# jonH34400/3DBodyAnimation

Measured on AMD Instinct MI355X. Metric: SMPL residual+Jacobian evals/sec (6890v, 10 beta, 24 joints), higher is better.
Workload: dtype f64 residual/Jacobian; f32 mesh (f32 + split-bf16 MFMA blend); 1 GPU; C3: 256 independent frames per GPU, BODY_25 (14 FK joints + 11 vertex landmarks), opt-shape (per-frame beta, 86 cols), GMM prior on, 6890-vertex mesh on; frames_per_gpu=256, keypoints_per_frame=25, n_cols=86

## Files before the change

3dbodyanimation_amd/csrc/frame_part_inl.h:

```cpp
#pragma once
#include <hip/hip_ext.h>

#include "bodyfit_device.h"
#include "priors_inl.h"

namespace bodyfit {
namespace {

__device__ __forceinline__ void store_through(double* p, double v) {
  __hip_atomic_store(p, v, __ATOMIC_RELAXED, __HIP_MEMORY_SCOPE_SYSTEM);
}
#ifndef BODYFIT_J_THROUGH
#define BODYFIT_J_THROUGH 1
#endif
template <bool kFused>
__device__ __forceinline__ void store_J(double* p, double v, int scope = 0) {
  if constexpr (kFused && !BODYFIT_J_THROUGH) *p = v;
  else if (scope == 1) store_f64_through(p, v);
  else if (scope == 2) *p = v;
  else store_through(p, v);
}


__device__ inline void mul33(const double* A, const double* B, double* C) {
#pragma unroll
  for (int r = 0; r < 3; ++r)
#pragma unroll
    for (int c = 0; c < 3; ++c) C[r * 3 + c] = A[r * 3] * B[c] + A[r * 3 + 1] * B[3 + c] + A[r * 3 + 2] * B[6 + c];
}
__device__ inline void mul33_bt(const double* A, const double* B, double* C) {
#pragma unroll
  for (int r = 0; r < 3; ++r)
#pragma unroll
    for (int c = 0; c < 3; ++c)
      C[r * 3 + c] = A[r * 3] * B[c * 3] + A[r * 3 + 1] * B[c * 3 + 1] + A[r * 3 + 2] * B[c * 3 + 2];
}
// ... 119 lines not shown
struct FusedFrame {
  unsigned* flag;
  unsigned epoch;
  int j_scope;
};

template <bool kFused>
__device__ __forceinline__ void frame_sync() {
  if constexpr (kFused) asm volatile("s_waitcnt lgkmcnt(0)\n\ts_barrier" ::: "memory");
  else __syncthreads();
}

template <bool kFused>
__device__ __forceinline__ void store_operand16(void* p, uint4 v) {
  if constexpr (kFused) {
    typedef __attribute__((ext_vector_type(4))) unsigned int u32x4_;
    const u32x4_ x = {v.x, v.y, v.z, v.w};
    asm volatile("global_store_dwordx4 %0, %1, off sc1\n\ts_nop 1" ::"v"(p), "v"(x) : "memory");
  } else {
    *reinterpret_cast<uint4*>(p) = v;
  }
}

template <bool kFused>
__device__ __forceinline__ void frame_part(const DevModel& M, const DevProblem& Pb, const double* __restrict__ params,
                                           const double* __restrict__ beta, double* __restrict__ r_out,
                                           double* __restrict__ J_out, double* __restrict__ joints_out, const MeshCoef& mc,
                                           int want_jac, double* sm, int f, const FusedFrame& fu, const FrameHead& hd) {
  const int tid = threadIdx.x;
  const int lane = tid & 63, wave = tid >> 6;
  const int nJ = kFused ? (hd.dims & 63) : M.nJ, nS = kFused ? ((hd.dims >> 6) & 15) : M.nS, nL = kFused ? ((hd.dims >> 10) & 63) : M.nL;
  const int ncols = kFused ? ((hd.dims >> 16) & 255) : Pb.ncols;
  const int npose = 7 + 3 * (nJ - 1);
  const bool use_shape = kFused ? (((hd.dims >> 24) & 1) != 0) : (Pb.use_shape != 0);
  const int beta_stride = kFused ? ((hd.dims >> 25) & 15) : Pb.beta_stride;
  const unsigned char* const mtab = kFused ? hd.mtab : M.tabA;
  const unsigned char* const ptab = kFused ? hd.ptab : Pb.ptab;
  const int* const t_parent = reinterpret_cast<const int*>(mtab + kTabParent);
  const unsigned* const t_anc = reinterpret_cast<const unsigned*>(mtab + kTabAnc);
  const unsigned long long* const t_chain = reinterpret_cast<const unsigned long long*>(mtab + kTabChain);
  const int* const t_lm_woff = reinterpret_cast<const int*>(mtab + kTabLmWoff);
  const int* const t_lm_wj = reinterpret_cast<const int*>(mtab + kTabLmWj);
  const double* const t_lm_ww = reinterpret_cast<const double*>(mtab + kTabLmWw);
  const double* const t_lm_vt = reinterpret_cast<const double*>(mtab + kTabLmVt);
  const double* const t_lm_sd = reinterpret_cast<const double*>(mtab + kTabLmSd);
  const double* const t_dS = reinterpret_cast<const double*>(mtab + kTabDS);
  const double* const t_Sc = reinterpret_cast<const double*>(mtab + kTabSc);
  const double* const t_offset = reinterpret_cast<const double*>(mtab + kTabOffset);
  const double* const t_Jc0 = reinterpret_cast<const double*>(mtab + kTabJc0);
  const int t_F = kFused ? hd.F : Pb.F, t_K = kFused ? hd.K : Pb.K;
  const int* const t_kp_offset = reinterpret_cast<const int*>(ptab);
  const int* const t_kp_id = reinterpret_cast<const int*>(ptab + ptab_id_off(t_F));
  const double* const t_kp_uv = reinterpret_cast<const double*>(ptab + ptab_uv_off(t_F, t_K));
  const double* const t_R0 = kFused ? hd.R0 : Pb.R0;
  const int P = M.P;
  double* sx = sm + OFF_X;
  double* sR = sm + OFF_R;
  double* sdR = sm + OFF_DR;
// ... 580 lines not shown
    }
  }
  double* sJb = sdR;
  double fold_acc = 0.0;
  typedef __attribute__((ext_vector_type(4))) double fold_d4;
  fold_d4 fold_gram = {0.0, 0.0, 0.0, 0.0};
  for (int kc0 = k_begin; kc0 < k_end; kc0 += KC) {
    const int nk = min(KC, k_end - kc0);
    frame_sync<kFused>();
    if (kc0 != k_begin) {
      if (tid < nk) stage_kp(tid, kc0);
      frame_sync<kFused>();
    }
    STAMP(7);
    if (want_jac) {
      const int njc = npose - 7;
      const int ngrp = kThreads / njc;
      if (tid < ngrp * njc) {
        const int g = tid / njc, kc = tid - g * njc, k = 1 + kc / 3;
        double Wm[9];
#pragma unroll
        for (int e9 = 0; e9 < 9; ++e9) Wm[e9] = sW[kc * 9 + e9];
        const double pk0 = sP[k * 3], pk1 = sP[k * 3 + 1], pk2 = sP[k * 3 + 2];
        for (int kk = g; kk < nk; kk += ngrp) {
          const int kg = kc0 + kk;
          const int id = sKpId[kk];
          const unsigned am = sKpAnc[kk];
          const double* kp = sKp + kk * 18;
          const double* G = kp + 12;
          double d0 = 0.0, d1 = 0.0, d2 = 0.0;
          if (id < nJ) {
            if ((am >> k) & 1u) {
              const double x0 = kp[0] - pk0, x1 = kp[1] - pk1, x2 = kp[2] - pk2;
              d0 = Wm[0] * x0 + Wm[1] * x1 + Wm[2] * x2;
              d1 = Wm[3] * x0 + Wm[4] * x1 + Wm[5] * x2;
              d2 = Wm[6] * x0 + Wm[7] * x1 + Wm[8] * x2;
            }
          } else {
            const double* o = sLm + (id - nJ) * LM_STRIDE + LM_PD + kc * 3;
            d0 = o[0]; d1 = o[1]; d2 = o[2];
          }
          store_J<kFused>(J_out + (size_t)(2 * kg) * ncols + 7 + kc, G[0] * d0 + G[1] * d1 + G[2] * d2, fu.j_scope);
          store_J<kFused>(J_out + (size_t)(2 * kg + 1) * ncols + 7 + kc, G[3] * d0 + G[4] * d1 + G[5] * d2, fu.j_scope);
        }
      }
      const int nsc = 7 + (ncols - npose);
      for (int e = tid; e < nk * nsc; e += kThreads) {
        const int kk = e / nsc, c = e - kk * nsc;
        const int kg = kc0 + kk;
        const int id = sKpId[kk];
        const double* kp = sKp + kk * 18;
        const double* G = kp + 12;
        double j0, j1;
        int col;
        if (c == 0) {
          col = 0;
          j0 = kp[6] * kp[3] + kp[7] * kp[4] + kp[8] * kp[5];
          j1 = kp[9] * kp[3] + kp[10] * kp[4] + kp[11] * kp[5];
        } else if (c < 4) {
          col = c;
          double t[3];
          mv3(dRr0 + (c - 1) * 9, kp[0], kp[1], kp[2], t);
          j0 = s * (kp[6] * t[0] + kp[7] * t[1] + kp[8] * t[2]);
          j1 = s * (kp[9] * t[0] + kp[10] * t[1] + kp[11] * t[2]);
        } else if (c < 7) {
          col = c;
          j0 = kp[6 + (c - 4)];
          j1 = kp[9 + (c - 4)];
        } else {
          const int k = c - 7;
          col = npose + k;
          double d0 = 0.0, d1 = 0.0, d2 = 0.0;
          if (use_shape) {
            if (id < nJ) {
              if (id == 0 || sParent[id] < 0) {
                d0 = sDS[(id * 3 + 0) * nS + k]; d1 = sDS[(id * 3 + 1) * nS + k]; d2 = sDS[(id * 3 + 2) * nS + k];
              } else {
                d0 = sB[(id * 3 + 0) * nS + k]; d1 = sB[(id * 3 + 1) * nS + k]; d2 = sB[(id * 3 + 2) * nS + k];
              }
            } else {
              const double* o = sLm + (id - nJ) * LM_STRIDE + LM_BETA + k * 3;
              d0 = o[0]; d1 = o[1]; d2 = o[2];
            }
          }
          j0 = G[0] * d0 + G[1] * d1 + G[2] * d2;
          j1 = G[3] * d0 + G[4] * d1 + G[5] * d2;
        }
        store_J<kFused>(J_out + (size_t)(2 * kg) * ncols + col, j0, fu.j_scope);
        store_J<kFused>(J_out + (size_t)(2 * kg + 1) * ncols + col, j1, fu.j_scope);
        if (fold && c >= 7) { sJb[(2 * kk) * kMaxShape + c - 7] = j0; sJb[(2 * kk + 1) * kMaxShape + c - 7] = j1; }
      }
    }
    if (fold) {
      frame_sync<kFused>();
      if (wave == 0) {
        const int col = lane & 15, kq = lane >> 4;
        for (int s0 = 0; s0 < (2 * nk + 3) / 4; s0 += 4) {
          double vv[4];
#pragma unroll
          for (int u = 0; u < 4; ++u) {
            const int row = 4 * (s0 + u) + kq;
            const bool on = row < 2 * nk;
            const double sw = on ? sFeat[row >> 1] : 0.0;
            const double x = (on && col < nS) ? sJb[row * kMaxShape + col] : ((on && col == 10) ? sKpUv[row] : 0.0);
            vv[u] = sw * x;
          }
#pragma unroll
          for (int u = 0; u < 4; ++u) fold_gram = __builtin_amdgcn_mfma_f64_16x16x4f64(vv[u], vv[u], fold_gram, 0, 0, 0);
        }
      } else if (tid == 64) {
        for (int kk = 0; kk < nk; ++kk) fold_acc += sFeat[KC + kk];
      }
    }
  }
// ... 24 lines not shown
```

3dbodyanimation_amd/csrc/k_sweep.hip:

```cpp
#include <hip/hip_ext.h>

#include "bodyfit_device.h"
#include "frame_part_inl.h"
#include "mesh_part_inl.h"
#include "mesh_role_inl.h"
#include "priors_inl.h"

namespace bodyfit {
namespace {

[[maybe_unused]] constexpr int kPollWave = 7;

__global__ __launch_bounds__(kThreads, 4) void k_frame_resjac(DevModel M, DevProblem Pb, const double* __restrict__ params,
                                                      const double* __restrict__ beta, double* __restrict__ r_out,
                                                      double* __restrict__ J_out, double* __restrict__ joints_out,
                                                      MeshCoef mc, int want_jac, PriorArgs pa) {
  extern __shared__ __attribute__((aligned(16))) double sm[];
  if ((int)blockIdx.x < pa.n_tiles) {
#ifdef BODYFIT_STAMPS
    unsigned long long tp0 = 0;
    if (Pb.dbg && threadIdx.x == 0) asm volatile("s_memrealtime %0\n\ts_waitcnt lgkmcnt(0)" : "=s"(tp0)::"memory");
#endif
    if (Pb.frame_flags) {
      const int f = (int)blockIdx.x * kPriorTileF + (int)(threadIdx.x & 15);
// ... 96 lines not shown
    out66[tid] = v;
  }
}

struct RoleArgs {
  DevModel M;
  DevProblem Pb;
  const double* params;
  const double* beta;
  double* r_out;
  double* J_out;
  double* joints_out;
  MeshCoef mc;
  int want_jac;
  PriorArgs pa;
  float* cloud_f;
  FusedSync sy;
  FoldTail fold;
};
typedef const __attribute__((address_space(4))) RoleArgs* RoleArgP;

static_assert(alignof(RoleArgs) == 8, "kernel-argument segment: 4 ints, 5 pointers, then RoleArgs at offset 56");
[[maybe_unused]] constexpr int kRoleArgsOffset = 4 * 4 + 5 * 8;
__global__ __launch_bounds__(kThreads, 4) void k_sweep_roles(int F_arg, int nVT_arg, int K_arg, int dims_arg,
                                                             const unsigned char* __restrict__ mtab_arg,
                                                             const unsigned char* __restrict__ ptab_arg,
                                                             const double* __restrict__ R0_arg, const double* __restrict__ params_arg,
                                                             const double* __restrict__ beta_arg, RoleArgs by_value) {
  (void)by_value;
#if defined(__HIP_DEVICE_COMPILE__)
  extern __shared__ __attribute__((aligned(16))) unsigned char lds[];
  const RoleArgP A =
      (RoleArgP)((const __attribute__((address_space(4))) unsigned char*)__builtin_amdgcn_kernarg_segment_ptr() + kRoleArgsOffset);
  const int F = F_arg, nVT = nVT_arg;
  int role = 2, idx = 0, grp = 0;
  {
    const int nG = (F + kRoleGroup - 1) / kRoleGroup;
    int pos = (int)blockIdx.x;
    const int n0 = min(kRoleGroup, F);
    if (pos < n0) { role = 0; idx = pos; }
    else {
      pos -= n0;
      bool found = false;
      for (int g = 1; g < nG && !found; ++g) {
        const int ng = min(kRoleGroup, F - kRoleGroup * g);
        if (pos < ng) { role = 0; idx = kRoleGroup * g + pos; found = true; }
        else {
          pos -= ng;
          if (pos < nVT) { role = 1; idx = pos; grp = g - 1; found = true; }
          else pos -= nVT;
        }
      }
      if (!found) {
        if (pos < nVT) { role = 1; idx = pos; grp = nG - 1; }
        else { role = 2; idx = pos - nVT; }
      }
    }
  }
  if (role == 0) {
    const DevModel M = A->M;
    const DevProblem Pb = A->Pb;
    const MeshCoef mc = A->mc;
    FusedFrame fu;
    fu.flag = A->sy.flag;
    fu.epoch = A->sy.epoch;
    fu.j_scope = A->sy.j_scope;
    __builtin_amdgcn_s_setprio(2);
    FrameHead hd;
    hd.mtab = mtab_arg; hd.ptab = ptab_arg; hd.R0 = R0_arg; hd.F = F_arg; hd.K = K_arg; hd.dims = dims_arg;
    frame_part<true>(M, Pb, params_arg, beta_arg, A->r_out, A->J_out, A->joints_out, mc, A->want_jac,
                     reinterpret_cast<double*>(lds), idx, fu, hd);
    if (A->fold.ticket)
      fold_tail(A->fold.ticket, A->fold.want, A->fold.n_partials, A->fold.partials, A->fold.beta, A->fold.shape_rows,
                A->fold.beta_shape, A->fold.out66, lds);
    return;
  }
  const unsigned epoch = A->sy.epoch;
  const unsigned long long kRoleTimeoutTicks = A->sy.timeout_ticks;
  unsigned* const flag_base = A->sy.flag;
  unsigned* const error_word = A->sy.error;
  if (role == 2) grp = (idx * kPriorTileF) / kRoleGroup;
  const unsigned max_polls = (unsigned)min(kRoleTimeoutTicks / 110ull, 0x7fffffffull);
  auto wait_flags = [&]() {
    const int tid = threadIdx.x, lane = tid & 63;
    if ((tid >> 6) == kPollWave) {
      const int fbeg = grp * kRoleGroup, nf = min(kRoleGroup, F - fbeg);
      const int nu = (nf + kFTile - 1) / kFTile;
      const unsigned want = epoch * (unsigned)min(kFTile, nf - min(lane, 7) * kFTile);
      const unsigned* ctr = flag_base + (size_t)(grp * (kRoleGroup / kFTile) + min(lane, 7)) * kUnitCounterStride;
      const unsigned long long t_enter = __builtin_amdgcn_s_memrealtime();
      for (unsigned polls = 0;; ++polls) {
        const unsigned got = __hip_atomic_load(ctr, __ATOMIC_RELAXED, __HIP_MEMORY_SCOPE_AGENT);
        if (__all(lane >= nu || got == want)) break;
        if (polls >= max_polls) break;
// ... 19 lines not shown
  const DevModel M = A->M;
  const DevProblem Pb = A->Pb;
  const MeshCoef mc = A->mc;
  const unsigned long long t_role = __builtin_amdgcn_s_memrealtime();
  const int my_unit = __builtin_amdgcn_readfirstlane(threadIdx.x >> 6);
  const unsigned want = epoch * (unsigned)max(0, min(kFTile, F - (grp * kRoleGroup + my_unit * kFTile)));
  const unsigned* ctr = flag_base + (size_t)(grp * (kRoleGroup / kFTile) + my_unit) * kUnitCounterStride;
  auto wait_unit = [&](const unsigned* c) -> bool {
    for (unsigned polls = 0;; ++polls) {
      const unsigned got = __hip_atomic_load(c, __ATOMIC_RELAXED, __HIP_MEMORY_SCOPE_AGENT);
      if (got == want) return true;
      if (polls >= max_polls) return false;
      if (__builtin_amdgcn_s_memrealtime() - t_role < 300) {
        for (int i = 0; i < 6 && __builtin_amdgcn_s_memrealtime() - t_role < 300; ++i) __builtin_amdgcn_s_sleep(20);
      } else {
        __builtin_amdgcn_s_sleep(9);
      }
    }
  };
  auto fail = [&]() {
    if (threadIdx.x == 0) __hip_atomic_store(error_word, 1u, __ATOMIC_RELAXED, __HIP_MEMORY_SCOPE_AGENT);
  };
  mesh_role(M, Pb, mc, A->cloud_f, idx, grp, lds, (int)blockIdx.x < A->sy.resident_blocks, ctr, want, wait_unit, fail,
            A->sy.mesh_prio_early, A->sy.trickle_start, A->sy.trickle_sleep);
#endif
}

}

void launch_frame_resjac(const DevModel& M, const DevProblem& P, const double* d_params, const double* d_beta,
                         double* d_r, double* d_J, double* d_joints, const MeshCoef& mc, int want_jac,
                         const PriorArgs& priors, hipStream_t s, hipEvent_t ev_start, hipEvent_t ev_stop) {
  if (P.F <= 0) return;
  const size_t lds = frame_lds_bytes(M.nL);
  static DeviceMax lds_granted;
  lds_granted.raise(current_device(), lds, 48 * 1024, [&](size_t want) {
    (void)hipFuncSetAttribute(reinterpret_cast<const void*>(k_frame_resjac), hipFuncAttributeMaxDynamicSharedMemorySize,
                              (int)want);
  });
  BODYFIT_LAUNCH_EXT(k_frame_resjac, dim3(P.F + priors.n_tiles), dim3(kThreads), lds, s, ev_start, ev_stop, 0, M, P,
                        d_params, d_beta, d_r, d_J, d_joints, mc, want_jac, priors);
}

void launch_mesh(const DevModel& M, const DevProblem& P, const MeshCoef& mc, float* d_cloud, const PriorArgs& pa,
                 const double* d_params, hipStream_t s, hipEvent_t ev_start, hipEvent_t ev_stop) {
  if (P.F <= 0) return;
  if ((size_t)P.nFTiles * kFTile * M.nVTiles * kVTile * 12 >= ((size_t)1 << 32)) return;
  static DeviceOnce attr;
  attr.run(current_device(), [&] {
    (void)hipFuncSetAttribute(reinterpret_cast<const void*>(k_mesh_blend_lbs),
                              hipFuncAttributeMaxDynamicSharedMemorySize, kLdsBytes);
  });
  BODYFIT_LAUNCH_EXT(k_mesh_blend_lbs, dim3(M.nVTiles + pa.n_tiles), dim3(64 * kWaves), kLdsBytes, s, ev_start, ev_stop,
                        0, M, P, mc, d_cloud, pa, d_params);
}

bool role_sweep_fits(const DevModel& M, const DevProblem& P) {
  return P.F > 0 && P.F <= kRoleMaxFrames && M.nVTiles > 0 && frame_lds_bytes(M.nL) <= (size_t)kRoleLdsBytes &&
         (size_t)P.nFTiles * kFTile * M.nVTiles * kVTile * 12 < ((size_t)1 << 32);
}

void launch_sweep_roles(const DevModel& M, const DevProblem& P, const double* d_params, const double* d_beta, double* d_r,
                        double* d_J, double* d_joints, const MeshCoef& mc, int want_jac, const PriorArgs& pa, float* d_cloud,
                        const FusedSync& sy, const FoldTail& fold, hipStream_t s, hipEvent_t ev_start, hipEvent_t ev_stop) {
  static DeviceOnce attr;
  attr.run(current_device(), [&] {
    (void)hipFuncSetAttribute(reinterpret_cast<const void*>(k_sweep_roles), hipFuncAttributeMaxDynamicSharedMemorySize,
                              kRoleLdsBytes);
  });
  const int nG = (P.F + kRoleGroup - 1) / kRoleGroup;
  const int grid = P.F + nG * M.nVTiles + pa.n_tiles;
  RoleArgs A;
  A.M = M; A.Pb = P; A.Pb.feat_perm = 1; A.params = d_params; A.beta = d_beta; A.r_out = d_r; A.J_out = d_J;
  A.joints_out = d_joints; A.mc = mc; A.want_jac = want_jac; A.pa = pa; A.cloud_f = d_cloud; A.sy = sy; A.fold = fold;
  const int dims = frame_head_dims(M.nJ, M.nS, M.nL, P.ncols, P.use_shape, P.beta_stride, mc.featA != nullptr);
  BODYFIT_LAUNCH_EXT(k_sweep_roles, dim3(grid), dim3(kThreads), kRoleLdsBytes, s, ev_start, ev_stop, 0, P.F, M.nVTiles, P.K, dims,
                     M.tabA, P.ptab, P.R0, d_params, d_beta, A);
}

}
```

3dbodyanimation_amd/csrc/mesh_role_inl.h:

```cpp
#pragma once
#include <hip/hip_ext.h>

#include "bodyfit_device.h"
#include "mesh_part_inl.h"

namespace bodyfit {
namespace {

constexpr int kRoleGroup = 256;
constexpr int kSlabBytes = 3 * 2 * 1024;
constexpr int kResident = 13;
constexpr int kRegionASlabs = 4;
constexpr int kRegionABytes = kRegionASlabs * kSlabBytes;
constexpr int kRegionTSlabs = kResident - kRegionASlabs;
constexpr int kTRowBytes = 2 * kRowBytes;
constexpr int kTRing = 4;
constexpr int kTWaveBytes = 3 * kTRowBytes;
constexpr int kTSlot3Bytes = kRegionABytes / kWaves;
constexpr int kRoleCtrlOff = kRegionABytes + kWaves * kTWaveBytes;
constexpr int kRoleLdsBytes = kRoleCtrlOff + 16;
constexpr int kLoadSc1 = 16;
static_assert(kRegionTSlabs * kSlabBytes == kWaves * kTWaveBytes, "the transform rings take over region T exactly");
static_assert(kTSlot3Bytes >= kTRowBytes, "ring slot 3");
static_assert(kRoleLdsBytes <= 80 * 1024, "two workgroups per CU");
__host__ __device__ constexpr int role_slab_off(int s) {
  return s < kRegionTSlabs ? kRegionABytes + s * kSlabBytes : (s - kRegionTSlabs) * kSlabBytes;
}

typedef __attribute__((address_space(3))) unsigned char lds_u8;
typedef __attribute__((ext_vector_type(4))) float f32x4;
typedef const __attribute__((address_space(3))) u32x4 lds_u32x4;
typedef const __attribute__((address_space(3))) f32x4 lds_f32x4;

#ifdef BODYFIT_STAMPS
#define RSTAMP(i)                                                                                              \
  do {                                                                                                         \
    if (Pb.dbg && C.lane == 0) {                                                                               \
      unsigned long long t_;                                                                                   \
      asm volatile("s_memrealtime %0\n\ts_waitcnt lgkmcnt(0)" : "=s"(t_)::"memory");                          \
      Pb.dbg[kStampBase + ((size_t)(group * M.nVTiles + vtile) * 8 + C.wave) * 16 + (i)] = t_;                 \
    }                                                                                                          \
  } while (0)
#define RCYC(i)                                                                                                \
  do {                                                                                                         \
// ... 31 lines not shown
};

__device__ __forceinline__ void role_dma_slab(const RoleCtx& C, int s) {
  __builtin_amdgcn_raw_ptr_buffer_load_lds(C.dirs_rsrc, (__attribute__((address_space(3))) void*)(C.ring + role_slab_off(s) + C.piece * 1024),
                                       16, C.slab_voff, C.dirs_soff + (unsigned)s * kSlabBytes, 0, 0);
}
__device__ __forceinline__ void role_dma_row(const RoleCtx& C, int r) {
  const unsigned so = C.skin_soff + (unsigned)r * kTRowBytes;
  lds_u8* l = (r % kTRing) == 3 ? C.trow3 : C.trow + (r % kTRing) * kTRowBytes;
  __builtin_amdgcn_raw_ptr_buffer_load_lds(C.skin_rsrc, (__attribute__((address_space(3))) void*)l, 16, C.lane * 16, so, 0, kLoadSc1);
  __builtin_amdgcn_raw_ptr_buffer_load_lds(C.skin_rsrc, (__attribute__((address_space(3))) void*)(l + 1024), 16, C.lane * 16, so + 1024, 0, kLoadSc1);
  __builtin_amdgcn_raw_ptr_buffer_load_lds(C.skin_rsrc, (__attribute__((address_space(3))) void*)(l + 2048), 4, C.lane * 4, so + 2048, 0, kLoadSc1);
}

template <int S>
__device__ __forceinline__ void role_blend_step(const RoleCtx& C, const __amdgpu_buffer_rsrc_t& feat_rsrc, unsigned feat_off,
                                                f32x16 (&acc)[3], u32x4 (&a)[3][2], u32x4 (&bq)[3][2]) {
  const bf16x8 a_hi = __builtin_bit_cast(bf16x8, a[S % 3][0]);
  const bf16x8 a_lo = __builtin_bit_cast(bf16x8, a[S % 3][1]);
#pragma unroll
  for (int c = 0; c < 3; ++c) {
    const bf16x8 bhi = __builtin_bit_cast(bf16x8, bq[c][0]);
    const bf16x8 blo = __builtin_bit_cast(bf16x8, bq[c][1]);
    if constexpr (S == 0) {
      f32x16 z;
#pragma unroll
      for (int r = 0; r < 16; ++r) z[r] = 0.0f;
      acc[c] = __builtin_amdgcn_mfma_f32_32x32x16_bf16(a_hi, bhi, z, 0, 0, 0);
    } else {
      acc[c] = __builtin_amdgcn_mfma_f32_32x32x16_bf16(a_hi, bhi, acc[c], 0, 0, 0);
    }
    acc[c] = __builtin_amdgcn_mfma_f32_32x32x16_bf16(a_hi, blo, acc[c], 0, 0, 0);
    acc[c] = __builtin_amdgcn_mfma_f32_32x32x16_bf16(a_lo, bhi, acc[c], 0, 0, 0);
    if constexpr (S + 1 < kResident && S + 1 != kRegionTSlabs) {
      const unsigned sl = C.ring_addr + (unsigned)(role_slab_off(S + 1) + (c * 2) * 1024);
      bq[c][0] = *(lds_u32x4*)(size_t)(sl);
      bq[c][1] = *(lds_u32x4*)(size_t)(sl + 1024u);
    } else if constexpr (S + 1 >= kResident && S + 1 < kBlendKSteps) {
      const unsigned so = C.dirs_soff + (unsigned)((S + 1) * kSlabBytes + (c * 2) * 1024);
      bq[c][0] = __builtin_amdgcn_raw_buffer_load_b128(C.dirs_rsrc, (unsigned)(C.lane * 16), so, 0);
      bq[c][1] = __builtin_amdgcn_raw_buffer_load_b128(C.dirs_rsrc, (unsigned)(C.lane * 16), so + 1024, 0);
    }
  }
  if constexpr (S + 3 < kBlendKSteps) {
    const unsigned soff = feat_off + (unsigned)((S + 3) * 2 * 1024);
    a[S % 3][0] = __builtin_amdgcn_raw_buffer_load_b128(feat_rsrc, feat_frag_off(C.lane, 0), soff, kLoadSc1);
    a[S % 3][1] = __builtin_amdgcn_raw_buffer_load_b128(feat_rsrc, feat_frag_off(C.lane, 1), soff, kLoadSc1);
  }
#pragma unroll
  for (int c = 0; c < 3; ++c) {
    __builtin_amdgcn_sched_group_barrier(0x008, 3, 0);
    if constexpr (S + 1 < kResident && S + 1 != kRegionTSlabs) __builtin_amdgcn_sched_group_barrier(0x100, 2, 0);
    else if constexpr (S + 1 >= kResident && S + 1 < kBlendKSteps) __builtin_amdgcn_sched_group_barrier(0x020, 2, 0);
  }
  if constexpr (S + 3 < kBlendKSteps) __builtin_amdgcn_sched_group_barrier(0x020, 2, 0);
  __builtin_amdgcn_sched_barrier(0);
}

template <int R>
__device__ __forceinline__ void role_skin_row(const RoleCtx& C, const RoleLane& L, const f32x16 (&acc)[3],
                                              __amdgpu_buffer_rsrc_t cloud, unsigned row_off) {
  if constexpr (R >= 3) ROLE_WAIT_VM(role_skin_ops(R - 3) + role_skin_ops(R - 2) + role_skin_ops(R - 1));
  const unsigned slot = (R % kTRing) == 3 ? L.slot3 : (unsigned)(R % kTRing) * kTRowBytes;
  f32x4 t[12];
  const unsigned tj[4] = {L.tj0, L.tj1, L.tj2, L.tj3};
  const float wgt[4] = {L.w0, L.w1, L.w2, L.w3};
#pragma unroll
  for (int i = 0; i < 4; ++i) {
    lds_f32x4* T = (lds_f32x4*)(tj[i] + slot);
    t[3 * i + 0] = T[0]; t[3 * i + 1] = T[1]; t[3 * i + 2] = T[2];
  }
  f32x2 b[6];
  const f32x2 w0 = {wgt[0], wgt[0]};
#pragma unroll
  for (int k = 0; k < 3; ++k) {
    b[2 * k] = w0 * f32x2{t[k].x, t[k].y};
    b[2 * k + 1] = w0 * f32x2{t[k].z, t[k].w};
  }
// ... 5 lines not shown
      b[2 * k] += wi * f32x2{t[3 * i + k].x, t[3 * i + k].y};
      b[2 * k + 1] += wi * f32x2{t[3 * i + k].z, t[3 * i + k].w};
    }
  }
  const f32x2 pxy = {acc[0][R], acc[1][R]};
  const f32x2 pz1 = {acc[2][R], 1.0f};
  typedef __attribute__((ext_vector_type(3))) unsigned int u32x3;
  u32x3 pk;
#pragma unroll
  for (int k = 0; k < 3; ++k) {
    const f32x2 m = b[2 * k] * pxy + b[2 * k + 1] * pz1;
    pk[k] = __float_as_uint(m.x + m.y);
  }
  __builtin_amdgcn_raw_buffer_store_b96(pk, cloud, L.out_off, row_off, kStoreAux);
  if constexpr (R + kTRing < 16) role_dma_row(C, R + kTRing);
  asm volatile("" ::: "memory");
}


template <typename WaitUnit, typename Fail>
__device__ __forceinline__ void mesh_role(const DevModel& M, const DevProblem& Pb, const MeshCoef& mc, float* __restrict__ cloud_f,
                                          int vtile, int group, unsigned char* lds_generic, bool beside_its_frames,
                                          const unsigned* unit_ctr, unsigned unit_want, WaitUnit wait_unit, Fail fail,
                                          int prio_early, int trickle_start, int trickle_sleep) {
  RoleCtx C;
  C.wave = __builtin_amdgcn_readfirstlane(threadIdx.x >> 6);
  C.lane = threadIdx.x & 63;
  lds_u8* lds = (lds_u8*)lds_generic;
  C.ring = lds;
  C.ring_addr = (unsigned)(size_t)lds + (unsigned)C.lane * 16u;
  C.trow = lds + kRegionABytes + C.wave * kTWaveBytes;
  C.trow3 = lds + C.wave * kTSlot3Bytes;
  C.dirs_rsrc = __builtin_amdgcn_make_buffer_rsrc(const_cast<uint16_t*>(M.dirsB), 0, M.nVTiles * kBBytes, 0x00020000);
  C.dirs_soff = (unsigned)vtile * kBBytes;
  const int nFT = Pb.nFTiles;
  const int ftile = group * (kRoleGroup / kFTile) + C.wave;
  const bool active = ftile < nFT;
  const int f0 = ftile * kFTile;
  C.skin_rsrc = __builtin_amdgcn_make_buffer_rsrc(mc.skinT, 0, nFT * kFTile * kRowBytes, 0x00020000);
  C.skin_soff = (unsigned)(active ? f0 : 0) * kRowBytes;
  C.piece = C.wave < 6 ? C.wave : C.wave - 6;
  C.slab_voff = C.piece * 1024 + C.lane * 16;
  const int col = C.lane & 31, h = C.lane >> 5;
  const int v = vtile * kVTile + col;
  RSTAMP(0);
  const uint32_t widx = M.wIdx[(size_t)vtile * 32 + col];
  const float4 wv = reinterpret_cast<const float4*>(M.wVal)[(size_t)vtile * 32 + col];
  if (C.wave < 6) {
    if (beside_its_frames) {
      const unsigned long long t_in = __builtin_amdgcn_s_memrealtime();
      while (__builtin_amdgcn_s_memrealtime() - t_in < (unsigned long long)trickle_start) __builtin_amdgcn_s_sleep(8);
    }
#pragma unroll 1
    for (int s = 0; s < kRegionTSlabs; ++s) {
      role_dma_slab(C, s);
      if (beside_its_frames)
        for (int z = 0; z < trickle_sleep; ++z) __builtin_amdgcn_s_sleep(1);
    }
  }
  RoleLane L;
  L.w0 = wv.x; L.w1 = wv.y; L.w2 = wv.z; L.w3 = wv.w;
  const unsigned trow_addr = (unsigned)(size_t)C.trow + (unsigned)h * kRowBytes;
  L.tj0 = trow_addr + (widx & 0xffu) * 48u;
  L.tj1 = trow_addr + ((widx >> 8) & 0xffu) * 48u;
  L.tj2 = trow_addr + ((widx >> 16) & 0xffu) * 48u;
  L.tj3 = trow_addr + (widx >> 24) * 48u;
  L.slot3 = (unsigned)(size_t)C.trow3 - (unsigned)(size_t)C.trow;
  const unsigned stride = (unsigned)M.nVTiles * kVTile * 12;
  L.out_off = (unsigned)h * stride + (unsigned)v * 12;
  const __amdgpu_buffer_rsrc_t cloud =
      __builtin_amdgcn_make_buffer_rsrc(cloud_f, 0, (int)((unsigned)nFT * kFTile * stride), 0x00020000);
  const unsigned feat_off = (unsigned)((active ? ftile : 0) * kBlendKSteps * 2 * 1024);

  volatile __attribute__((address_space(3))) unsigned* ctrl =
      (volatile __attribute__((address_space(3))) unsigned*)(lds + kRoleCtrlOff);
  if (threadIdx.x == 0) ctrl[0] = 0u;
  __builtin_amdgcn_s_waitcnt(0x0F70);
  asm volatile("s_waitcnt lgkmcnt(0)\n\ts_barrier" ::: "memory");
  if (active && !wait_unit(unit_ctr + kUnitCoefOffset)) ctrl[0] = 1u;
  RSTAMP(1);
  if (prio_early == 0) __builtin_amdgcn_s_setprio(0);
  else if (prio_early == 1) __builtin_amdgcn_s_setprio(1);
  else if (prio_early == 2) __builtin_amdgcn_s_setprio(2);
  else __builtin_amdgcn_s_setprio(3);

  f32x16 acc[3];
  u32x4 a[3][2], bq[3][2];
  const __amdgpu_buffer_rsrc_t feat_rsrc =
      __builtin_amdgcn_make_buffer_rsrc(mc.featA, 0, nFT * kBlendKSteps * 2 * 1024, 0x00020000);
  RSTAMP(2);
#define RB(S) RCYC(S); role_blend_step<S>(C, feat_rsrc, feat_off, acc, a, bq)
  unsigned look1 = unit_want;
  if (active) {
#pragma unroll
    for (int ks = 0; ks < 3; ++ks) {
      const unsigned soff = feat_off + (unsigned)(ks * 2 * 1024);
      a[ks][0] = __builtin_amdgcn_raw_buffer_load_b128(feat_rsrc, feat_frag_off(C.lane, 0), soff, kLoadSc1);
      a[ks][1] = __builtin_amdgcn_raw_buffer_load_b128(feat_rsrc, feat_frag_off(C.lane, 1), soff, kLoadSc1);
    }
    __builtin_amdgcn_sched_barrier(0);
#pragma unroll
    for (int s = kRegionTSlabs; s < kResident; ++s) role_dma_slab(C, s);
    __builtin_amdgcn_sched_barrier(0);
#pragma unroll
    for (int c = 0; c < 3; ++c) {
      const unsigned sl = C.ring_addr + (unsigned)(role_slab_off(0) + (c * 2) * 1024);
      bq[c][0] = *(lds_u32x4*)(size_t)(sl);
      bq[c][1] = *(lds_u32x4*)(size_t)(sl + 1024u);
    }
    RB(0); RB(1); RB(2); RB(3); RB(4); RB(5); RB(6);
    asm volatile("global_load_dword %0, %1, off sc1" : "=v"(look1) : "v"(unit_ctr) : "memory");
    RB(7); RB(8);
    asm volatile("s_waitcnt vmcnt(5)" ::: "memory");
  } else {
#pragma unroll
    for (int s = kRegionTSlabs; s < kResident; ++s) role_dma_slab(C, s);
    asm volatile("s_waitcnt vmcnt(0)" ::: "memory");
  }
  asm volatile("s_waitcnt lgkmcnt(0)\n\ts_barrier" ::: "memory");
  if (active) {
#pragma unroll
    for (int c = 0; c < 3; ++c) {
      const unsigned sl = C.ring_addr + (unsigned)(role_slab_off(kRegionTSlabs) + (c * 2) * 1024);
      bq[c][0] = *(lds_u32x4*)(size_t)(sl);
      bq[c][1] = *(lds_u32x4*)(size_t)(sl + 1024u);
    }
    RB(9); RB(10);
    asm volatile("s_waitcnt vmcnt(8)" : "+v"(look1)::"memory");
    if (look1 != unit_want && !wait_unit(unit_ctr)) ctrl[0] = 1u;
    else { role_dma_row(C, 0); role_dma_row(C, 1); role_dma_row(C, 2); }
    asm volatile("" ::: "memory");
    __builtin_amdgcn_s_setprio(3);
    RB(11); RB(12); RB(13);
  }
#undef RB
  RCYC(14);
  __builtin_amdgcn_sched_barrier(0);
  asm volatile("s_waitcnt lgkmcnt(0)\n\ts_barrier" ::: "memory");
  __builtin_amdgcn_sched_barrier(0);
  if (ctrl[0] != 0u) {
    asm volatile("s_waitcnt vmcnt(0)" ::: "memory");
    fail();
    return;
  }
  if (!active) return;
  RSTAMP(3);
  role_dma_row(C, 3);
  asm volatile("" ::: "memory");
  ROLE_WAIT_VM(3);
  const unsigned row0 = (unsigned)f0 * stride;
#define RS(R) RCYC(16 + (R)); role_skin_row<R>(C, L, acc, cloud, row0 + (unsigned)(2 * (R)) * stride)
  RS(0); RS(1); RS(2); RS(3); RS(4); RS(5); RS(6); RS(7); RS(8); RS(9); RS(10); RS(11); RS(12); RS(13); RS(14); RS(15);
#undef RS
  RCYC(32);
  RSTAMP(4);
}
// ... 4 lines not shown
```

Baseline: 12.33 million evals/s.

## Specialize frame kernel for SMPL dims and split Jacobian column work by role

Adds a compile-time FrameDimsSmpl specialization of the sweep kernel, selected at launch when the dimensions match, so loop bounds and strides become constants. The per-joint pose Jacobian loop now prefetches the next keypoint's LDS data one iteration ahead. The shape and rigid columns are split across disjoint whole-wave thread groups, with branch-free selects replacing the divergent per-column branches. It also adds an optional, default-off path that computes the pose-free beta k-step from directly loaded betas before the other blend steps. The cost is an extra kernel instantiation and more code-path variants to keep consistent.

```diff
diff --git a/3dbodyanimation_amd/csrc/frame_part_inl.h b/3dbodyanimation_amd/csrc/frame_part_inl.h
--- a/3dbodyanimation_amd/csrc/frame_part_inl.h
+++ b/3dbodyanimation_amd/csrc/frame_part_inl.h
@@ -12,6 +12,9 @@
 }
 #ifndef BODYFIT_J_THROUGH
 #define BODYFIT_J_THROUGH 1
+#endif
+#ifndef BODYFIT_F2_BATCH
+#define BODYFIT_F2_BATCH 1
 #endif
 template <bool kFused>
 __device__ __forceinline__ void store_J(double* p, double v, int scope = 0) {
@@ -177,18 +180,37 @@
   }
 }
 
-template <bool kFused>
+#ifndef BODYFIT_FIXED_SHAPE
+#define BODYFIT_FIXED_SHAPE 1
+#endif
+struct FrameDimsRuntime {
+  static constexpr bool kFixed = false;
+  static constexpr int nJ = 0, nS = 0, nL = 0, ncols = 0, beta_stride = 0;
+  static constexpr bool use_shape = false;
+};
+struct FrameDimsSmpl {
+  static constexpr bool kFixed = true;
+  static constexpr int nJ = 24, nS = 10, nL = 11, ncols = 86, beta_stride = 10;
+  static constexpr bool use_shape = true;
+  __host__ __device__ static bool matches(int nJ_, int nS_, int nL_, int ncols_, int use_shape_, int beta_stride_) {
+    return nJ_ == nJ && nS_ == nS && nL_ == nL && ncols_ == ncols && use_shape_ != 0 && beta_stride_ == beta_stride;
+  }
+};
+
+template <bool kFused, typename Dims = FrameDimsRuntime>
 __device__ __forceinline__ void frame_part(const DevModel& M, const DevProblem& Pb, const double* __restrict__ params,
                                            const double* __restrict__ beta, double* __restrict__ r_out,
                                            double* __restrict__ J_out, double* __restrict__ joints_out, const MeshCoef& mc,
                                            int want_jac, double* sm, int f, const FusedFrame& fu, const FrameHead& hd) {
   const int tid = threadIdx.x;
   const int lane = tid & 63, wave = tid >> 6;
-  const int nJ = kFused ? (hd.dims & 63) : M.nJ, nS = kFused ? ((hd.dims >> 6) & 15) : M.nS, nL = kFused ? ((hd.dims >> 10) & 63) : M.nL;
-  const int ncols = kFused ? ((hd.dims >> 16) & 255) : Pb.ncols;
+  constexpr bool kFix = Dims::kFixed;
+  const int nJ = kFix ? Dims::nJ : (kFused ? (hd.dims & 63) : M.nJ), nS = kFix ? Dims::nS : (kFused ? ((hd.dims >> 6) & 15) : M.nS),
+            nL = kFix ? Dims::nL : (kFused ? ((hd.dims >> 10) & 63) : M.nL);
+  const int ncols = kFix ? Dims::ncols : (kFused ? ((hd.dims >> 16) & 255) : Pb.ncols);
   const int npose = 7 + 3 * (nJ - 1);
-  const bool use_shape = kFused ? (((hd.dims >> 24) & 1) != 0) : (Pb.use_shape != 0);
-  const int beta_stride = kFused ? ((hd.dims >> 25) & 15) : Pb.beta_stride;
+  const bool use_shape = kFix ? Dims::use_shape : (kFused ? (((hd.dims >> 24) & 1) != 0) : (Pb.use_shape != 0));
+  const int beta_stride = kFix ? Dims::beta_stride : (kFused ? ((hd.dims >> 25) & 15) : Pb.beta_stride);
   const unsigned char* const mtab = kFused ? hd.mtab : M.tabA;
   const unsigned char* const ptab = kFused ? hd.ptab : Pb.ptab;
   const int* const t_parent = reinterpret_cast<const int*>(mtab + kTabParent);
@@ -815,6 +837,47 @@
 #pragma unroll
         for (int e9 = 0; e9 < 9; ++e9) Wm[e9] = sW[kc * 9 + e9];
         const double pk0 = sP[k * 3], pk1 = sP[k * 3 + 1], pk2 = sP[k * 3 + 2];
+#if BODYFIT_F2_BATCH
+        struct KpStage { unsigned am; double q0, q1, q2, G[6], o0, o1, o2; };
+        auto kp_fetch = [&](int kk_, int id_) {
+          KpStage n;
+          const double* kp_ = sKp + kk_ * 18;
+          n.am = sKpAnc[kk_];
+          n.q0 = kp_[0]; n.q1 = kp_[1]; n.q2 = kp_[2];
+#pragma unroll
+          for (int i = 0; i < 6; ++i) n.G[i] = kp_[12 + i];
+          n.o0 = 0.0; n.o1 = 0.0; n.o2 = 0.0;
+          if (id_ >= nJ) {
+            const double* o = sLm + (id_ - nJ) * LM_STRIDE + LM_PD + kc * 3;
+            n.o0 = o[0]; n.o1 = o[1]; n.o2 = o[2];
+          }
+          return n;
+        };
+        int id_nx = sKpId[min(g, nk - 1)];
+        KpStage nx = kp_fetch(min(g, nk - 1), id_nx);
+        int id_nx2 = sKpId[min(g + ngrp, nk - 1)];
+        for (int kk = g; kk < nk; kk += ngrp) {
+          const int kg = kc0 + kk;
+          const KpStage cu = nx;
+          const int id = id_nx;
+          id_nx = id_nx2;
+          nx = kp_fetch(min(kk + ngrp, nk - 1), id_nx);
+          id_nx2 = sKpId[min(kk + 2 * ngrp, nk - 1)];
+          double d0 = 0.0, d1 = 0.0, d2 = 0.0;
+          if (id < nJ) {
+            if ((cu.am >> k) & 1u) {
+              const double x0 = cu.q0 - pk0, x1 = cu.q1 - pk1, x2 = cu.q2 - pk2;
+              d0 = Wm[0] * x0 + Wm[1] * x1 + Wm[2] * x2;
+              d1 = Wm[3] * x0 + Wm[4] * x1 + Wm[5] * x2;
+              d2 = Wm[6] * x0 + Wm[7] * x1 + Wm[8] * x2;
+            }
+          } else {
+            d0 = cu.o0; d1 = cu.o1; d2 = cu.o2;
+          }
+          store_J<kFused>(J_out + (size_t)(2 * kg) * ncols + 7 + kc, cu.G[0] * d0 + cu.G[1] * d1 + cu.G[2] * d2, fu.j_scope);
+          store_J<kFused>(J_out + (size_t)(2 * kg + 1) * ncols + 7 + kc, cu.G[3] * d0 + cu.G[4] * d1 + cu.G[5] * d2, fu.j_scope);
+        }
+#else
         for (int kk = g; kk < nk; kk += ngrp) {
           const int kg = kc0 + kk;
           const int id = sKpId[kk];
@@ -836,7 +899,59 @@
           store_J<kFused>(J_out + (size_t)(2 * kg) * ncols + 7 + kc, G[0] * d0 + G[1] * d1 + G[2] * d2, fu.j_scope);
           store_J<kFused>(J_out + (size_t)(2 * kg + 1) * ncols + 7 + kc, G[3] * d0 + G[4] * d1 + G[5] * d2, fu.j_scope);
         }
-      }
+#endif
+      }
+#if BODYFIT_F2_BATCH
+      constexpr int kShapeThreads = KC * kMaxShape;
+      static_assert(kShapeThreads % 64 == 0 && kShapeThreads < kThreads, "F2: whole waves per kind of column");
+      const int nshape = ncols - npose;
+      if (tid < kShapeThreads) {
+        for (int e = tid; e < nk * nshape; e += kShapeThreads) {
+          const int kk = e / nshape, k = e - kk * nshape;
+          const int kg = kc0 + kk;
+          const int id = sKpId[kk];
+          const double* G = sKp + kk * 18 + 12;
+          const double G0 = G[0], G1 = G[1], G2 = G[2], G3 = G[3], G4 = G[4], G5 = G[5];
+          const bool is_joint = id < nJ;
+          const int idj = is_joint ? id : 0;
+          const int par = sParent[idj];
+          const double* pa_ = is_joint ? (sB + (idj * 3) * nS + k) : (sLm + (id - nJ) * LM_STRIDE + LM_BETA + k * 3);
+          const int st_ = is_joint ? nS : 1;
+          const double a0 = pa_[0], a1 = pa_[st_], a2 = pa_[2 * st_];
+          const double r0 = sDS[(idj * 3 + 0) * nS + k], r1 = sDS[(idj * 3 + 1) * nS + k], r2 = sDS[(idj * 3 + 2) * nS + k];
+          const bool rootish = is_joint && (id == 0 || par < 0);
+          const double d0 = use_shape ? (rootish ? r0 : a0) : 0.0, d1 = use_shape ? (rootish ? r1 : a1) : 0.0,
+                       d2 = use_shape ? (rootish ? r2 : a2) : 0.0;
+          const double j0 = G0 * d0 + G1 * d1 + G2 * d2;
+          const double j1 = G3 * d0 + G4 * d1 + G5 * d2;
+          store_J<kFused>(J_out + (size_t)(2 * kg) * ncols + npose + k, j0, fu.j_scope);
+          store_J<kFused>(J_out + (size_t)(2 * kg + 1) * ncols + npose + k, j1, fu.j_scope);
+          if (fold) { sJb[(2 * kk) * kMaxShape + k] = j0; sJb[(2 * kk + 1) * kMaxShape + k] = j1; }
+        }
+      } else {
+        for (int e = tid - kShapeThreads; e < nk * 7; e += kThreads - kShapeThreads) {
+          const int kk = e / 7, c = e - kk * 7;
+          const int kg = kc0 + kk;
+          const double* kp = sKp + kk * 18;
+          double q[12];
+#pragma unroll
+          for (int i = 0; i < 12; ++i) q[i] = kp[i];
+          const int cr = min(max(c - 1, 0), 2), ct = min(max(c - 4, 0), 2);
+          double t[3];
+          mv3(dRr0 + cr * 9, q[0], q[1], q[2], t);
+          const double sc0 = q[6] * q[3] + q[7] * q[4] + q[8] * q[5];
+          const double sc1 = q[9] * q[3] + q[10] * q[4] + q[11] * q[5];
+          const double ro0 = s * (q[6] * t[0] + q[7] * t[1] + q[8] * t[2]);
+          const double ro1 = s * (q[9] * t[0] + q[10] * t[1] + q[11] * t[2]);
+          const double tr0 = ct == 0 ? q[6] : (ct == 1 ? q[7] : q[8]);
+          const double tr1 = ct == 0 ? q[9] : (ct == 1 ? q[10] : q[11]);
+          const double j0 = c == 0 ? sc0 : (c < 4 ? ro0 : tr0);
+          const double j1 = c == 0 ? sc1 : (c < 4 ? ro1 : tr1);
+          store_J<kFused>(J_out + (size_t)(2 * kg) * ncols + c, j0, fu.j_scope);
+          store_J<kFused>(J_out + (size_t)(2 * kg + 1) * ncols + c, j1, fu.j_scope);
+        }
+      }
+#else
       const int nsc = 7 + (ncols - npose);
       for (int e = tid; e < nk * nsc; e += kThreads) {
         const int kk = e / nsc, c = e - kk * nsc;
@@ -883,6 +998,7 @@
         store_J<kFused>(J_out + (size_t)(2 * kg + 1) * ncols + col, j1, fu.j_scope);
         if (fold && c >= 7) { sJb[(2 * kk) * kMaxShape + c - 7] = j0; sJb[(2 * kk + 1) * kMaxShape + c - 7] = j1; }
       }
+#endif
     }
     if (fold) {
       frame_sync<kFused>();
diff --git a/3dbodyanimation_amd/csrc/k_sweep.hip b/3dbodyanimation_amd/csrc/k_sweep.hip
--- a/3dbodyanimation_amd/csrc/k_sweep.hip
+++ b/3dbodyanimation_amd/csrc/k_sweep.hip
@@ -1,4 +1,6 @@
 #include <hip/hip_ext.h>
+
+#include <cstdlib>
 
 #include "bodyfit_device.h"
 #include "frame_part_inl.h"
@@ -142,6 +144,7 @@
 
 static_assert(alignof(RoleArgs) == 8, "kernel-argument segment: 4 ints, 5 pointers, then RoleArgs at offset 56");
 [[maybe_unused]] constexpr int kRoleArgsOffset = 4 * 4 + 5 * 8;
+template <typename FrameDims>
 __global__ __launch_bounds__(kThreads, 4) void k_sweep_roles(int F_arg, int nVT_arg, int K_arg, int dims_arg,
                                                              const unsigned char* __restrict__ mtab_arg,
                                                              const unsigned char* __restrict__ ptab_arg,
@@ -188,8 +191,8 @@
     __builtin_amdgcn_s_setprio(2);
     FrameHead hd;
     hd.mtab = mtab_arg; hd.ptab = ptab_arg; hd.R0 = R0_arg; hd.F = F_arg; hd.K = K_arg; hd.dims = dims_arg;
-    frame_part<true>(M, Pb, params_arg, beta_arg, A->r_out, A->J_out, A->joints_out, mc, A->want_jac,
-                     reinterpret_cast<double*>(lds), idx, fu, hd);
+    frame_part<true, FrameDims>(M, Pb, params_arg, beta_arg, A->r_out, A->J_out, A->joints_out, mc, A->want_jac,
+                                reinterpret_cast<double*>(lds), idx, fu, hd);
     if (A->fold.ticket)
       fold_tail(A->fold.ticket, A->fold.want, A->fold.n_partials, A->fold.partials, A->fold.beta, A->fold.shape_rows,
                 A->fold.beta_shape, A->fold.out66, lds);
@@ -255,7 +258,8 @@
     if (threadIdx.x == 0) __hip_atomic_store(error_word, 1u, __ATOMIC_RELAXED, __HIP_MEMORY_SCOPE_AGENT);
   };
   mesh_role(M, Pb, mc, A->cloud_f, idx, grp, lds, (int)blockIdx.x < A->sy.resident_blocks, ctr, want, wait_unit, fail,
-            A->sy.mesh_prio_early, A->sy.trickle_start, A->sy.trickle_sleep);
+            A->sy.mesh_prio_early, A->sy.trickle_start, A->sy.trickle_sleep,
+            beta_arg, (dims_arg >> 25) & 15, (((dims_arg >> 24) & 1) != 0 && beta_arg != nullptr) ? ((dims_arg >> 6) & 15) : 0, F);
 #endif
 }
 
@@ -298,8 +302,12 @@
                         const FusedSync& sy, const FoldTail& fold, hipStream_t s, hipEvent_t ev_start, hipEvent_t ev_stop) {
   static DeviceOnce attr;
   attr.run(current_device(), [&] {
-    (void)hipFuncSetAttribute(reinterpret_cast<const void*>(k_sweep_roles), hipFuncAttributeMaxDynamicSharedMemorySize,
-                              kRoleLdsBytes);
+    (void)hipFuncSetAttribute(reinterpret_cast<const void*>(k_sweep_roles<FrameDimsRuntime>),
+                              hipFuncAttributeMaxDynamicSharedMemorySize, kRoleLdsBytes);
+#if BODYFIT_FIXED_SHAPE
+    (void)hipFuncSetAttribute(reinterpret_cast<const void*>(k_sweep_roles<FrameDimsSmpl>),
+                              hipFuncAttributeMaxDynamicSharedMemorySize, kRoleLdsBytes);
+#endif
   });
   const int nG = (P.F + kRoleGroup - 1) / kRoleGroup;
   const int grid = P.F + nG * M.nVTiles + pa.n_tiles;
@@ -307,8 +315,16 @@
   A.M = M; A.Pb = P; A.Pb.feat_perm = 1; A.params = d_params; A.beta = d_beta; A.r_out = d_r; A.J_out = d_J;
   A.joints_out = d_joints; A.mc = mc; A.want_jac = want_jac; A.pa = pa; A.cloud_f = d_cloud; A.sy = sy; A.fold = fold;
   const int dims = frame_head_dims(M.nJ, M.nS, M.nL, P.ncols, P.use_shape, P.beta_stride, mc.featA != nullptr);
-  BODYFIT_LAUNCH_EXT(k_sweep_roles, dim3(grid), dim3(kThreads), kRoleLdsBytes, s, ev_start, ev_stop, 0, P.F, M.nVTiles, P.K, dims,
-                     M.tabA, P.ptab, P.R0, d_params, d_beta, A);
-}
-
-}
+#if BODYFIT_FIXED_SHAPE
+  const char* generic = std::getenv("BODYFIT_SWEEP_GENERIC");
+  if (FrameDimsSmpl::matches(M.nJ, M.nS, M.nL, P.ncols, P.use_shape, P.beta_stride) && !(generic && generic[0] == '1')) {
+    BODYFIT_LAUNCH_EXT(k_sweep_roles<FrameDimsSmpl>, dim3(grid), dim3(kThreads), kRoleLdsBytes, s, ev_start, ev_stop, 0, P.F,
+                       M.nVTiles, P.K, dims, M.tabA, P.ptab, P.R0, d_params, d_beta, A);
+    return;
+  }
+#endif
+  BODYFIT_LAUNCH_EXT(k_sweep_roles<FrameDimsRuntime>, dim3(grid), dim3(kThreads), kRoleLdsBytes, s, ev_start, ev_stop, 0, P.F,
+                     M.nVTiles, P.K, dims, M.tabA, P.ptab, P.R0, d_params, d_beta, A);
+}
+
+}
diff --git a/3dbodyanimation_amd/csrc/mesh_role_inl.h b/3dbodyanimation_amd/csrc/mesh_role_inl.h
--- a/3dbodyanimation_amd/csrc/mesh_role_inl.h
+++ b/3dbodyanimation_amd/csrc/mesh_role_inl.h
@@ -20,6 +20,12 @@
 constexpr int kRoleCtrlOff = kRegionABytes + kWaves * kTWaveBytes;
 constexpr int kRoleLdsBytes = kRoleCtrlOff + 16;
 constexpr int kLoadSc1 = 16;
+#ifndef BODYFIT_POSE_FREE_FIRST
+#define BODYFIT_POSE_FREE_FIRST 0
+#endif
+constexpr int kPoseFreeStep = kBlendKSteps - 1;
+constexpr int kBlendBehind = BODYFIT_POSE_FREE_FIRST ? kPoseFreeStep : kBlendKSteps;
+static_assert(16 * kPoseFreeStep > kPoseFeat, "the last k-step holds no pose feature");
 static_assert(kRegionTSlabs * kSlabBytes == kWaves * kTWaveBytes, "the transform rings take over region T exactly");
 static_assert(kTSlot3Bytes >= kTRowBytes, "ring slot 3");
 static_assert(kRoleLdsBytes <= 80 * 1024, "two workgroups per CU");
@@ -97,7 +103,7 @@
   for (int c = 0; c < 3; ++c) {
     const bf16x8 bhi = __builtin_bit_cast(bf16x8, bq[c][0]);
     const bf16x8 blo = __builtin_bit_cast(bf16x8, bq[c][1]);
-    if constexpr (S == 0) {
+    if constexpr (S == 0 && !BODYFIT_POSE_FREE_FIRST) {
       f32x16 z;
 #pragma unroll
       for (int r = 0; r < 16; ++r) z[r] = 0.0f;
@@ -111,13 +117,13 @@
       const unsigned sl = C.ring_addr + (unsigned)(role_slab_off(S + 1) + (c * 2) * 1024);
       bq[c][0] = *(lds_u32x4*)(size_t)(sl);
       bq[c][1] = *(lds_u32x4*)(size_t)(sl + 1024u);
-    } else if constexpr (S + 1 >= kResident && S + 1 < kBlendKSteps) {
+    } else if constexpr (S + 1 >= kResident && S + 1 < kBlendBehind) {
       const unsigned so = C.dirs_soff + (unsigned)((S + 1) * kSlabBytes + (c * 2) * 1024);
       bq[c][0] = __builtin_amdgcn_raw_buffer_load_b128(C.dirs_rsrc, (unsigned)(C.lane * 16), so, 0);
       bq[c][1] = __builtin_amdgcn_raw_buffer_load_b128(C.dirs_rsrc, (unsigned)(C.lane * 16), so + 1024, 0);
     }
   }
-  if constexpr (S + 3 < kBlendKSteps) {
+  if constexpr (S + 3 < kBlendBehind) {
     const unsigned soff = feat_off + (unsigned)((S + 3) * 2 * 1024);
     a[S % 3][0] = __builtin_amdgcn_raw_buffer_load_b128(feat_rsrc, feat_frag_off(C.lane, 0), soff, kLoadSc1);
     a[S % 3][1] = __builtin_amdgcn_raw_buffer_load_b128(feat_rsrc, feat_frag_off(C.lane, 1), soff, kLoadSc1);
@@ -126,9 +132,9 @@
   for (int c = 0; c < 3; ++c) {
     __builtin_amdgcn_sched_group_barrier(0x008, 3, 0);
     if constexpr (S + 1 < kResident && S + 1 != kRegionTSlabs) __builtin_amdgcn_sched_group_barrier(0x100, 2, 0);
-    else if constexpr (S + 1 >= kResident && S + 1 < kBlendKSteps) __builtin_amdgcn_sched_group_barrier(0x020, 2, 0);
-  }
-  if constexpr (S + 3 < kBlendKSteps) __builtin_amdgcn_sched_group_barrier(0x020, 2, 0);
+    else if constexpr (S + 1 >= kResident && S + 1 < kBlendBehind) __builtin_amdgcn_sched_group_barrier(0x020, 2, 0);
+  }
+  if constexpr (S + 3 < kBlendBehind) __builtin_amdgcn_sched_group_barrier(0x020, 2, 0);
   __builtin_amdgcn_sched_barrier(0);
 }
 
@@ -180,7 +186,8 @@
 __device__ __forceinline__ void mesh_role(const DevModel& M, const DevProblem& Pb, const MeshCoef& mc, float* __restrict__ cloud_f,
                                           int vtile, int group, unsigned char* lds_generic, bool beside_its_frames,
                                           const unsigned* unit_ctr, unsigned unit_want, WaitUnit wait_unit, Fail fail,
-                                          int prio_early, int trickle_start, int trickle_sleep) {
+                                          int prio_early, int trickle_start, int trickle_sleep,
+                                          const double* __restrict__ beta, int beta_stride, int n_beta, int F) {
   RoleCtx C;
   C.wave = __builtin_amdgcn_readfirstlane(threadIdx.x >> 6);
   C.lane = threadIdx.x & 63;
@@ -204,11 +211,44 @@
   RSTAMP(0);
   const uint32_t widx = M.wIdx[(size_t)vtile * 32 + col];
   const float4 wv = reinterpret_cast<const float4*>(M.wVal)[(size_t)vtile * 32 + col];
-  if (C.wave < 6) {
+#if BODYFIT_POSE_FREE_FIRST
+  u32x4 a13[2];
+  {
+    typedef __attribute__((ext_vector_type(2))) unsigned int u32x2_;
+    u32x2_ beta_raw[8];
+    const int pf_row = C.lane & 31, pf_half = C.lane >> 5;
+    const int pf_frame = f0 + 8 * (pf_row >> 3) + 2 * (pf_row & 3) + ((pf_row >> 2) & 1);
+    const bool pf_beta = active && n_beta > 0 && pf_frame < F;
+    const __amdgpu_buffer_rsrc_t beta_rsrc = __builtin_amdgcn_make_buffer_rsrc(
+        const_cast<double*>(beta), 0, n_beta > 0 ? (int)(((unsigned)(F - 1) * (unsigned)beta_stride + (unsigned)n_beta) * 8u) : 0, 0x00020000);
+    const unsigned frame_off = (unsigned)min(active ? pf_frame : 0, F - 1) * (unsigned)beta_stride * 8u;
+#pragma unroll
+    for (int u = 0; u < 8; ++u)
+      beta_raw[u] = __builtin_amdgcn_raw_buffer_load_b64(beta_rsrc, frame_off + (unsigned)min(1 + 8 * pf_half + u, max(n_beta, 1) - 1) * 8u, 0, 0);
     if (beside_its_frames) {
       const unsigned long long t_in = __builtin_amdgcn_s_memrealtime();
       while (__builtin_amdgcn_s_memrealtime() - t_in < (unsigned long long)trickle_start) __builtin_amdgcn_s_sleep(8);
     }
+#pragma unroll
+    for (int q = 0; q < 4; ++q) {
+      uint32_t hi2 = 0u, lo2 = 0u;
+#pragma unroll
+      for (int t = 0; t < 2; ++t) {
+        const int i = 1 + 8 * pf_half + 2 * q + t;
+        const double bd = __longlong_as_double((long long)(((unsigned long long)beta_raw[2 * q + t].y << 32) |
+                                                            (unsigned long long)beta_raw[2 * q + t].x));
+        const float x = (pf_beta && i < n_beta) ? (float)bd : ((i == kMaxShape || i == kMaxShape + 1) ? 1.0f : 0.0f);
+        const uint16_t hi = f32_to_bf16(x);
+        const uint16_t lo = f32_to_bf16(x - bf16_to_f32(hi));
+        hi2 |= (uint32_t)hi << (16 * t);
+        lo2 |= (uint32_t)lo << (16 * t);
+      }
+      a13[0][q] = hi2;
+      a13[1][q] = lo2;
+    }
+    __builtin_amdgcn_s_waitcnt(0x0F70);
+  }
+  if (C.wave < 6) {
 #pragma unroll 1
     for (int s = 0; s < kRegionTSlabs; ++s) {
       role_dma_slab(C, s);
@@ -216,6 +256,21 @@
         for (int z = 0; z < trickle_sleep; ++z) __builtin_amdgcn_s_sleep(1);
     }
   }
+#else
+  if (C.wave < 6) {
+    if (beside_its_frames) {
+      const unsigned long long t_in = __builtin_amdgcn_s_memrealtime();
+      while (__builtin_amdgcn_s_memrealtime() - t_in < (unsigned long long)trickle_start) __builtin_amdgcn_s_sleep(8);
+    }
+#pragma unroll 1
+    for (int s = 0; s < kRegionTSlabs; ++s) {
+      role_dma_slab(C, s);
+      if (beside_its_frames)
+        for (int z = 0; z < trickle_sleep; ++z) __builtin_amdgcn_s_sleep(1);
+    }
+  }
+#endif
+  RSTAMP(5);
   RoleLane L;
   L.w0 = wv.x; L.w1 = wv.y; L.w2 = wv.z; L.w3 = wv.w;
   const unsigned trow_addr = (unsigned)(size_t)C.trow + (unsigned)h * kRowBytes;
@@ -234,7 +289,10 @@
       (volatile __attribute__((address_space(3))) unsigned*)(lds + kRoleCtrlOff);
   if (threadIdx.x == 0) ctrl[0] = 0u;
   __builtin_amdgcn_s_waitcnt(0x0F70);
+  RSTAMP(6);
+  f32x16 acc[3];
   asm volatile("s_waitcnt lgkmcnt(0)\n\ts_barrier" ::: "memory");
+  RSTAMP(7);
   if (active && !wait_unit(unit_ctr + kUnitCoefOffset)) ctrl[0] = 1u;
   RSTAMP(1);
   if (prio_early == 0) __builtin_amdgcn_s_setprio(0);
@@ -242,7 +300,6 @@
   else if (prio_early == 2) __builtin_amdgcn_s_setprio(2);
   else __builtin_amdgcn_s_setprio(3);
 
-  f32x16 acc[3];
   u32x4 a[3][2], bq[3][2];
   const __amdgpu_buffer_rsrc_t feat_rsrc =
       __builtin_amdgcn_make_buffer_rsrc(mc.featA, 0, nFT * kBlendKSteps * 2 * 1024, 0x00020000);
@@ -250,6 +307,15 @@
 #define RB(S) RCYC(S); role_blend_step<S>(C, feat_rsrc, feat_off, acc, a, bq)
   unsigned look1 = unit_want;
   if (active) {
+#if BODYFIT_POSE_FREE_FIRST
+#pragma unroll
+    for (int c = 0; c < 3; ++c) {
+      const unsigned so = C.dirs_soff + (unsigned)(kPoseFreeStep * kSlabBytes + (c * 2) * 1024);
+      bq[c][0] = __builtin_amdgcn_raw_buffer_load_b128(C.dirs_rsrc, (unsigned)(C.lane * 16), so, 0);
+      bq[c][1] = __builtin_amdgcn_raw_buffer_load_b128(C.dirs_rsrc, (unsigned)(C.lane * 16), so + 1024, 0);
+    }
+    __builtin_amdgcn_sched_barrier(0);
+#endif
 #pragma unroll
     for (int ks = 0; ks < 3; ++ks) {
       const unsigned soff = feat_off + (unsigned)(ks * 2 * 1024);
@@ -260,12 +326,39 @@
 #pragma unroll
     for (int s = kRegionTSlabs; s < kResident; ++s) role_dma_slab(C, s);
     __builtin_amdgcn_sched_barrier(0);
+#if BODYFIT_POSE_FREE_FIRST
+    {
+      const bf16x8 a_hi = __builtin_bit_cast(bf16x8, a13[0]);
+      const bf16x8 a_lo = __builtin_bit_cast(bf16x8, a13[1]);
+#pragma unroll
+      for (int c = 0; c < 3; ++c) {
+        const bf16x8 bhi = __builtin_bit_cast(bf16x8, bq[c][0]);
+        const bf16x8 blo = __builtin_bit_cast(bf16x8, bq[c][1]);
+        f32x16 z;
+#pragma unroll
+        for (int r = 0; r < 16; ++r) z[r] = 0.0f;
+        acc[c] = __builtin_amdgcn_mfma_f32_32x32x16_bf16(a_hi, bhi, z, 0, 0, 0);
+        acc[c] = __builtin_amdgcn_mfma_f32_32x32x16_bf16(a_hi, blo, acc[c], 0, 0, 0);
+        acc[c] = __builtin_amdgcn_mfma_f32_32x32x16_bf16(a_lo, bhi, acc[c], 0, 0, 0);
+        const unsigned sl = C.ring_addr + (unsigned)(role_slab_off(0) + (c * 2) * 1024);
+        bq[c][0] = *(lds_u32x4*)(size_t)(sl);
+        bq[c][1] = *(lds_u32x4*)(size_t)(sl + 1024u);
+      }
+#pragma unroll
+      for (int c = 0; c < 3; ++c) {
+        __builtin_amdgcn_sched_group_barrier(0x008, 3, 0);
+        __builtin_amdgcn_sched_group_barrier(0x100, 2, 0);
+      }
+      __builtin_amdgcn_sched_barrier(0);
+    }
+#else
 #pragma unroll
     for (int c = 0; c < 3; ++c) {
       const unsigned sl = C.ring_addr + (unsigned)(role_slab_off(0) + (c * 2) * 1024);
       bq[c][0] = *(lds_u32x4*)(size_t)(sl);
       bq[c][1] = *(lds_u32x4*)(size_t)(sl + 1024u);
     }
+#endif
     RB(0); RB(1); RB(2); RB(3); RB(4); RB(5); RB(6);
     asm volatile("global_load_dword %0, %1, off sc1" : "=v"(look1) : "v"(unit_ctr) : "memory");
     RB(7); RB(8);
@@ -284,12 +377,17 @@
       bq[c][1] = *(lds_u32x4*)(size_t)(sl + 1024u);
     }
     RB(9); RB(10);
-    asm volatile("s_waitcnt vmcnt(8)" : "+v"(look1)::"memory");
+    asm volatile("s_waitcnt vmcnt(%1)" : "+v"(look1) : "n"(BODYFIT_POSE_FREE_FIRST ? 6 : 8) : "memory");
     if (look1 != unit_want && !wait_unit(unit_ctr)) ctrl[0] = 1u;
     else { role_dma_row(C, 0); role_dma_row(C, 1); role_dma_row(C, 2); }
     asm volatile("" ::: "memory");
     __builtin_amdgcn_s_setprio(3);
-    RB(11); RB(12); RB(13);
+    RB(11); RB(12);
+#if !BODYFIT_POSE_FREE_FIRST
+    RB(13);
+#else
+    RCYC(13);
+#endif
   }
 #undef RB
   RCYC(14);
```

Result: faster. 12.52 million evals/s, median of 6 (+1.5%).
